# vwxyzjn/cleanrl

Hardware: NVIDIA H100
Metric: env steps/sec (SPS) PPO Breakout num_envs=1024 (higher is better)
Workload: dtype bf16

## Files before the change

cleanrl_b200/csrc/tc_conv1_u8.cuh:

```cuda
#pragma once
#include "tc_base.cuh"
#include <cuda_fp16.h>
#include "tc_conv_win.cuh"

namespace b200rl {
using namespace tc;

__device__ __forceinline__ uint64_t desc_kmajor_sw64(uint32_t smem_addr) {
    return (uint64_t)((smem_addr & 0x3FFFFu) >> 4) | (1ull << 16) | (32ull << 32) | kDescSwizzle64;
}
__device__ __forceinline__ uint64_t desc_mnmajor_sw64(uint32_t smem_addr, uint32_t lbo) {
    return (uint64_t)((smem_addr & 0x3FFFFu) >> 4) | ((uint64_t)((lbo >> 4) & 0x3FFF) << 16) | (32ull << 32) | kDescSwizzle64;
}
__device__ __forceinline__ uint32_t img64_off(int r, int c) { return (uint32_t)(r * 64 + ((c ^ ((r >> 1) & 3)) << 4)); }
constexpr int kS2dThreads = 256;
__global__ void __launch_bounds__(kS2dThreads) tc_frames_to_s2d_u8(const uint8_t* __restrict__ obs, const int64_t* __restrict__ rows,
                                                                   int64_t n, uint8_t* __restrict__ out_rm, uint8_t* __restrict__ out_cm) {
    __shared__ __align__(16) uint8_t frame[28224];
    const int64_t i = blockIdx.x;
    const int64_t img = rows ? rows[i] : i;
    const int4* src = reinterpret_cast<const int4*>(obs + img * 28224);
#pragma unroll
    for (int k = 0; k < 7; ++k) {
        const int t = threadIdx.x + k * kS2dThreads;
        if (t < 1764) reinterpret_cast<int4*>(frame)[t] = __ldg(src + t);
    }
    __syncthreads();
    int4* rm = reinterpret_cast<int4*>(out_rm + i * 441 * 64);
    for (int t = threadIdx.x; t < 441 * 4; t += kS2dThreads) {
        const int pos = t >> 2, c = t & 3;
        const int Y = (pos * 3121) >> 16, X = pos - Y * 21;
        const uint8_t* p = frame + c * 7056 + (Y * 4) * 84 + X * 4;
        int4 v;
        v.x = *reinterpret_cast<const int*>(p); v.y = *reinterpret_cast<const int*>(p + 84);
        v.z = *reinterpret_cast<const int*>(p + 168); v.w = *reinterpret_cast<const int*>(p + 252);
        rm[t] = v;
    }
    uint8_t* cm = out_cm + i * 64 * 448;
    for (int t = threadIdx.x; t < 16 * 112; t += kS2dThreads) {
        const int g = t / 112, q = t - g * 112;
        const uint8_t* prow = frame + (g >> 2) * 7056 + (g & 3) * 84;
        uint32_t w[4];
#pragma unroll
        for (int e = 0; e < 4; ++e) {
            const int pos = q * 4 + e, pc = pos < 441 ? pos : 440;
            const int Y = (pc * 3121) >> 16, X = pc - Y * 21;
            const uint32_t v = *reinterpret_cast<const uint32_t*>(prow + (Y * 4) * 84 + X * 4);
            w[e] = pos < 441 ? v : 0u;
        }
        const uint32_t lo01 = __byte_perm(w[0], w[1], 0x5140), hi01 = __byte_perm(w[0], w[1], 0x7362);
        const uint32_t lo23 = __byte_perm(w[2], w[3], 0x5140), hi23 = __byte_perm(w[2], w[3], 0x7362);
        uint32_t* dst = reinterpret_cast<uint32_t*>(cm + (g * 4) * 448) + q;
        dst[0] = __byte_perm(lo01, lo23, 0x5410);
        dst[112] = __byte_perm(lo01, lo23, 0x7632);
        dst[224] = __byte_perm(hi01, hi23, 0x5410);
        dst[336] = __byte_perm(hi01, hi23, 0x7632);
    }
}

__global__ void __launch_bounds__(256) tc_pack_conv1_i8(const float* __restrict__ w, int8_t* __restrict__ limbs, float* __restrict__ sc) {
    __shared__ float red[32];
    const int co = blockIdx.x, idx = threadIdx.x;
    const float v = w[co * 256 + idx];
    float m = fabsf(v);
#pragma unroll
    for (int o = 16; o > 0; o >>= 1) m = fmaxf(m, __shfl_xor_sync(0xffffffffu, m, o));
    if ((idx & 31) == 0) red[idx >> 5] = m;
    __syncthreads();
    float mx = red[0];
#pragma unroll
    for (int k = 1; k < 8; ++k) mx = fmaxf(mx, red[k]);
    const float s = mx > 0.f ? mx * (128.0f / 127.0f) : 1.0f;
    const float u = v / s * 128.0f;
    float l1 = rintf(u);
    l1 = fminf(fmaxf(l1, -127.f), 127.f);
    float l2 = rintf((u - l1) * 128.0f);
    l2 = fminf(fmaxf(l2, -127.f), 127.f);
    const int kx = idx & 7, ky = (idx >> 3) & 7, c = idx >> 6;
    const int a = ky >> 2, sy = ky & 3, b = kx >> 2, sx = kx & 3;
    const int k = (a * 2 + b) * 64 + c * 16 + sy * 4 + sx;
    limbs[co * 256 + k] = (int8_t)l1;
    limbs[(32 + co) * 256 + k] = (int8_t)l2;
    if (idx == 0) {
        sc[co] = s / 128.0f / 255.0f;
        sc[32 + co] = s / 16384.0f / 255.0f;
    }
}

struct Conv1U8Params {
    const int64_t* rows;
    int n;
    int64_t n_images;
    const int8_t* limbs;
    const float* sc;
    const float* bias;
    bf16* out;
    uint32_t* mask_out;
};

constexpr int kConv1I8Threads = 384;
template <int STAGES>
__global__ void __launch_bounds__(kConv1I8Threads, 1) tc_conv1_i8(const __grid_constant__ CUtensorMap tmA, const __grid_constant__ CUtensorMap tmW,
                                                                   const Conv1U8Params p, int total_tiles) {
    constexpr int BN = 64, WR = 144, NTAPS = 4;
    constexpr int STAGE_BYTES = WR * 128;
    constexpr int B_CHUNK = BN * 64;
    extern __shared__ uint8_t smem_raw[];
    __shared__ uint64_t full_bar[STAGES], empty_bar[STAGES], w_bar;
    __shared__ __align__(16) float s_sc[32], s_bias[32];
    uint8_t* smem = reinterpret_cast<uint8_t*>((reinterpret_cast<uintptr_t>(smem_raw) + 1023) & ~uintptr_t(1023));
    const int tid = threadIdx.x, warp = tid >> 5;
    uint8_t* sW = smem;
    uint8_t* sRing = smem + NTAPS * B_CHUNK;

    if (tid == 0) {
        for (int s = 0; s < STAGES; ++s) { mbar_init(&full_bar[s], 1); mbar_init(&empty_bar[s], 8); }
        mbar_init(&w_bar, 1);
        fence_barrier_init();
        tma_prefetch_desc(&tmA);
        tma_prefetch_desc(&tmW);
    }
    if (tid < 32) { s_sc[tid] = p.sc[32 + tid]; s_bias[tid] = p.bias[tid]; }
    __syncthreads();
    const int tile_begin = (int)(((int64_t)total_tiles * blockIdx.x) / gridDim.x);
    const int tile_end = (int)(((int64_t)total_tiles * (blockIdx.x + 1)) / gridDim.x);

    if (warp == 0) {
        if (tid == 0) {
            uint32_t q = 0;
            int z_next = 0;
            if (tile_begin < tile_end) {
                const int img = tile_begin >> 1;
                z_next = p.rows ? (int)__ldg(p.rows + img) : img;
            }
            for (int tile = tile_begin; tile < tile_end; ++tile, ++q) {
                const uint32_t s = q % STAGES;
                const int z = z_next;
                if (tile + 1 < tile_end) {
                    const int img = (tile + 1) >> 1;
                    z_next = p.rows ? (int)__ldg(p.rows + img) : img;
                }
                if (q >= (uint32_t)STAGES) mbar_wait(&empty_bar[s], ((q / STAGES) - 1) & 1);
                mbar_arrive_expect_tx(&full_bar[s], (uint32_t)STAGE_BYTES);
                tma_load_3d(smem_u32(sRing + (size_t)s * STAGE_BYTES), &tmA, 0, (tile & 1) * 128, z, &full_bar[s]);
                if (q == 0) {
                    mbar_arrive_expect_tx(&w_bar, (uint32_t)(NTAPS * B_CHUNK));
#pragma unroll
                    for (int t = 0; t < NTAPS; ++t) tma_load_3d(smem_u32(sW + t * B_CHUNK), &tmW, t * 64, 0, 0, &w_bar);
                }
            }
        }
    } else if (warp >= 4) {
        const int wg = (warp - 4) >> 2, wt = tid & 127, lane = tid & 31, qd = lane & 3;
        const uint32_t w_base = smem_u32(sW);
        constexpr int off[4] = {0, 1, 21, 22};
        int acc[2][32];
#pragma unroll
        for (int e = 0; e < 2; ++e)
#pragma unroll
            for (int c = 0; c < 32; ++c) acc[e][c] = 0;
        if (tile_begin < tile_end) mbar_wait(&w_bar, 0);
        for (int tile = tile_begin; tile < tile_end; ++tile) {
            const uint32_t q = (uint32_t)(tile - tile_begin), s = q % STAGES;
            mbar_wait(&full_bar[s], (q / STAGES) & 1);
            wgmma_fence();
            const uint32_t win = smem_u32(sRing + (size_t)s * STAGE_BYTES) + (uint32_t)(wg * 64 * 128);
#pragma unroll
            for (int e = 0; e < 2; ++e) {
#pragma unroll
                for (int t = 0; t < NTAPS; ++t) {
                    const int po = e + off[t];
                    const uint64_t a = desc_kmajor(win + (uint32_t)((po >> 1) * 128 + (po & 1) * 64));
                    const uint64_t b = desc_kmajor_sw64(w_base + (uint32_t)(t * B_CHUNK));
#pragma unroll
                    for (int kk = 0; kk < 2; ++kk) wgmma_u8s8_n64(acc[e], a + 2 * kk, b + 2 * kk, (t | kk) != 0 ? 1u : 0u);
                }
            }
            wgmma_commit();
            wgmma_wait<0>();
            wgmma_fence_operands(acc[0]);
            wgmma_fence_operands(acc[1]);
            if (lane == 0) mbar_arrive(&empty_bar[s]);
            const int i = tile >> 1;
#pragma unroll
            for (int e = 0; e < 2; ++e) {
#pragma unroll
                for (int hr = 0; hr < 2; ++hr) {
                    const int lrow = wg * 64 + ((wt >> 5) << 4) + (lane >> 2) + 8 * hr;
                    const int rem = 2 * (((tile & 1) << 7) + lrow) + e;
                    const int Y = (rem * 3121) >> 16, X = rem - Y * 21;
                    const bool valid = rem < 441 && Y < 20 && X < 20;
                    const int64_t cell = ((int64_t)i * 10 + (Y >> 1)) * 10 + (X >> 1);
                    const int cls = (Y & 1) * 2 + (X & 1);
                    uint32_t bits = 0u, pk[4];
#pragma unroll
                    for (int j = 0; j < 4; ++j) {
                        const int co = 8 * j + 2 * qd;
                        const float f0 = fmaf((float)(acc[e][4 * j + 2 * hr] * 128 + acc[e][4 * (j + 4) + 2 * hr]), s_sc[co], s_bias[co]);
                        const float f1 = fmaf((float)(acc[e][4 * j + 2 * hr + 1] * 128 + acc[e][4 * (j + 4) + 2 * hr + 1]), s_sc[co + 1],
                                              s_bias[co + 1]);
                        bits |= (f0 > 0.f ? 1u : 0u) << co;
                        bits |= (f1 > 0.f ? 1u : 0u) << (co + 1);
                        pk[j] = pack_bf16x2_relu(f0, f1);
                    }
                    bits |= __shfl_xor_sync(0xffffffffu, bits, 1);
                    bits |= __shfl_xor_sync(0xffffffffu, bits, 2);
                    if (valid) {
                        if (qd == 0) p.mask_out[cell * 4 + cls] = bits;
                        uint32_t* dst = reinterpret_cast<uint32_t*>(reinterpret_cast<uint8_t*>(p.out) + (cell * 4 + cls) * 64);
#pragma unroll
                        for (int j = 0; j < 4; ++j) dst[4 * j + qd] = pk[j];
                    }
                }
            }
        }
    }
}

struct Conv21BwdU8Params {
    const int64_t* rows;
    int n;
    int64_t rows_per_cta;
    const bf16* w2dg;
    const uint32_t* m1;
    float* ws;
    float* wsb;
};
constexpr int kC1WXStages = 4, kC21WinStages = 2;
constexpr int kC1WXRows = 33, kC1WXBytes = kC1WXRows * 128, kC1WF16Bytes = 136 * 128;
constexpr int kC1WYBytes = 128 * 64, kC1WYPadRows = 24, kC1WYPad = kC1WYPadRows * 64;
constexpr int kC1WShift = 21;
constexpr int kC21WinRows = 140, kC21WinBytes = 18 * 1024;
constexpr int kC21W2Bytes = 4 * 128 * 128;
constexpr int kC21ImgBytes = kC1WYPad + 4 * kC1WYBytes;
constexpr int kC21MaskBytes = 100 * 16;
constexpr size_t kC21Smem = (size_t)kC21W2Bytes + (size_t)kC21WinStages * (kC21WinBytes + kC21MaskBytes) + 2 * (size_t)kC21ImgBytes +
                            2 * (size_t)kC1WF16Bytes + (size_t)kC1WXStages * kC1WXBytes + 1024;
static_assert(kC21Smem + 4608 <= 227 * 1024, "conv21_bwd: shared memory exceeds 227 KB");
static_assert((kC21W2Bytes + kC21WinStages * kC21WinBytes + 2 * kC21ImgBytes) % 1024 == 0, "the fp16 images need 1 KB alignment");
constexpr float kDact1Scale = 4096.0f;

__device__ __forceinline__ uint32_t prmt(uint32_t a, uint32_t b, uint32_t sel) {
    uint32_t d;
    asm("prmt.b32 %0, %1, %2, %3;" : "=r"(d) : "r"(a), "r"(b), "r"(sel));
    return d;
}
constexpr float kU8Bias = 1024.0f;
__device__ __forceinline__ void u8x16_to_f16_biased(const uint4& v, uint4& lo, uint4& hi) {
    constexpr uint32_t k64 = 0x64646464u;
    lo = make_uint4(prmt(v.x, k64, 0x5140u), prmt(v.x, k64, 0x7362u), prmt(v.y, k64, 0x5140u), prmt(v.y, k64, 0x7362u));
    hi = make_uint4(prmt(v.z, k64, 0x5140u), prmt(v.z, k64, 0x7362u), prmt(v.w, k64, 0x5140u), prmt(v.w, k64, 0x7362u));
}
__device__ __forceinline__ uint4 lds128(uint32_t addr) {
    uint4 v;
    asm volatile("ld.shared.v4.u32 {%0, %1, %2, %3}, [%4];" : "=r"(v.x), "=r"(v.y), "=r"(v.z), "=r"(v.w) : "r"(addr) : "memory");
    return v;
}
__device__ __forceinline__ void sts128(uint32_t addr, const uint4& v) {
    asm volatile("st.shared.v4.u32 [%0], {%1, %2, %3, %4};" ::"r"(addr), "r"(v.x), "r"(v.y), "r"(v.z), "r"(v.w) : "memory");
}
__device__ __forceinline__ uint32_t pack_f16x2_sat(float lo, float hi) {
    uint32_t d;
    asm("cvt.rn.satfinite.f16x2.f32 %0, %1, %2;" : "=r"(d) : "f"(hi), "f"(lo));
    return d;
}

__device__ __forceinline__ void sts32(uint32_t addr, uint32_t v) { asm volatile("st.shared.u32 [%0], %1;" ::"r"(addr), "r"(v) : "memory"); }
__device__ __forceinline__ void tma_store_3d(const void* tmap, uint32_t smem_src, int x, int y, int z) {
    asm volatile("cp.async.bulk.tensor.3d.global.shared::cta.bulk_group [%0, {%1, %2, %3}], [%4];"
                 ::"l"(reinterpret_cast<uint64_t>(tmap)), "r"(x), "r"(y), "r"(z), "r"(smem_src) : "memory");
}
__device__ __forceinline__ void bulk_commit() { asm volatile("cp.async.bulk.commit_group;" ::: "memory"); }
template <int N> __device__ __forceinline__ void bulk_wait_read() { asm volatile("cp.async.bulk.wait_group.read %0;" ::"n"(N) : "memory"); }
template <int N> __device__ __forceinline__ void bulk_wait() { asm volatile("cp.async.bulk.wait_group %0;" ::"n"(N) : "memory"); }
__device__ __forceinline__ void bulk_load(uint32_t smem_dst, const void* src, uint32_t bytes, uint64_t* bar) {
    asm volatile("cp.async.bulk.shared::cluster.global.mbarrier::complete_tx::bytes [%0], [%1], %2, [%3];"
                 ::"r"(smem_dst), "l"(src), "r"(bytes), "r"(smem_u32(bar)) : "memory");
}

constexpr int kC1WThreads = 512;
__global__ void __launch_bounds__(kC1WThreads, 1) tc_conv21_bwd_u8(const __grid_constant__ CUtensorMap tmX, const __grid_constant__ CUtensorMap tmWin,
                                                                 const __grid_constant__ CUtensorMap tmY, const Conv21BwdU8Params p) {
    constexpr int XS = kC1WXStages, WS = kC21WinStages;
    extern __shared__ uint8_t smem_raw[];
    __shared__ uint64_t xfull[XS], xempty[XS], wfull[WS], wempty[WS], yfull[2], yempty[2], ffull[2], fempty[2];
    __shared__ float sRed[32 * 32], sBias[32];
    uint8_t* smem = reinterpret_cast<uint8_t*>((reinterpret_cast<uintptr_t>(smem_raw) + 1023) & ~uintptr_t(1023));
    uint8_t* sW2 = smem;
    uint8_t* sWin = sW2 + kC21W2Bytes;
    uint8_t* sImg = sWin + (size_t)WS * kC21WinBytes;
    uint8_t* sF = sImg + 2 * (size_t)kC21ImgBytes;
    uint8_t* sX = sF + 2 * (size_t)kC1WF16Bytes;
    uint8_t* sM = sX + (size_t)XS * kC1WXBytes;
    const int tid = threadIdx.x, warp = tid >> 5, lane = tid & 31;
    if (tid == 0) {
        for (int s = 0; s < XS; ++s) { mbar_init(&xfull[s], 1); mbar_init(&xempty[s], 4); }
        for (int s = 0; s < WS; ++s) { mbar_init(&wfull[s], 1); mbar_init(&wempty[s], 4); }
        for (int s = 0; s < 2; ++s) {
            mbar_init(&yfull[s], 1); mbar_init(&yempty[s], 4);
            mbar_init(&ffull[s], 4); mbar_init(&fempty[s], 4);
        }
        fence_barrier_init();
        tma_prefetch_desc(&tmX);
        tma_prefetch_desc(&tmWin);
        tma_prefetch_desc(&tmY);
    }
    for (int idx = tid; idx < 4 * 128 * 8; idx += blockDim.x) {
        const int c16 = idx & 7, r = (idx >> 3) & 127, t = idx >> 10;
        *reinterpret_cast<int4*>(sW2 + t * (128 * 128) + img_off(r, c16)) = ldg16(p.w2dg + r * 256 + t * 64 + c16 * 8);
    }
    for (int idx = tid; idx < 2 * kC21ImgBytes / 16; idx += blockDim.x) reinterpret_cast<int4*>(sImg)[idx] = make_int4(0, 0, 0, 0);
    fence_proxy_async_smem();
    __syncthreads();
    const int64_t M = (int64_t)p.n * 512;
    const int64_t m_begin = (int64_t)blockIdx.x * p.rows_per_cta;
    int64_t m_end = m_begin + p.rows_per_cta;
    if (m_end > M) m_end = M;
    const int nsteps = (int)((m_end - m_begin) >> 7);
    const int nimg = nsteps >> 2;
    const int img0 = (int)(m_begin >> 9);

    if (warp < 4) {
        if (warp == 0 && lane == 0) {
            auto image_of = [&](int j) -> int { return p.rows ? (int)__ldg(p.rows + img0 + j) : img0 + j; };
            int z = 0, z_next = image_of(0);
            for (int k = 0; k < nsteps; ++k) {
                if ((k & 3) == 0) {
                    z = z_next;
                    if ((k >> 2) + 1 < nimg) z_next = image_of((k >> 2) + 1);
                }
#pragma unroll
                for (int hb = 0; hb < 2; ++hb) {
                    const int j = 2 * k + hb, xs = j % XS;
                    if (j >= XS) mbar_wait(&xempty[xs], ((j / XS) - 1) & 1);
                    mbar_arrive_expect_tx(&xfull[xs], (uint32_t)kC1WXBytes);
                    tma_load_3d(smem_u32(sX + (size_t)xs * kC1WXBytes), &tmX, 0, (k & 3) * 64 + hb * 32, z, &xfull[xs]);
                }
            }
        } else if (warp == 1 && lane == 0) {
            for (int j = 0; j < nimg; ++j) {
                const int s = j % WS;
                if (j >= WS) mbar_wait(&wempty[s], ((j / WS) - 1) & 1);
                mbar_arrive_expect_tx(&wfull[s], (uint32_t)(kC21WinRows * 128 + kC21MaskBytes));
                tma_load_2d(smem_u32(sWin + (size_t)s * kC21WinBytes), &tmWin, 0, (img0 + j) * 121, &wfull[s]);
                bulk_load(smem_u32(sM + (size_t)s * kC21MaskBytes), p.m1 + (int64_t)(img0 + j) * 100 * 4, (uint32_t)kC21MaskBytes, &wfull[s]);
            }
        }
    } else if (warp < 8) {
        const int wt = tid - 128, lane4 = lane >> 2, qd = lane & 3;
        const uint32_t w_base = smem_u32(sW2);
        const int rq = wt >> 2, c16 = wt & 3;
        float bsum[8];
#pragma unroll
        for (int e = 0; e < 8; ++e) bsum[e] = 0.f;
        for (int j = 0; j < nimg; ++j) {
            const int i = img0 + j, buf = j & 1, s = j % WS;
            const uint32_t img = smem_u32(sImg + (size_t)buf * kC21ImgBytes) + kC1WYPad;
            const uint32_t masks = smem_u32(sM + (size_t)s * kC21MaskBytes);
            mbar_wait(&wfull[s], (j / WS) & 1);
            if (j >= 2) mbar_wait(&yempty[buf], ((j >> 1) - 1) & 1);
            if (wt == 0) bulk_wait_read<1>();
            named_bar(1, 128);
#pragma unroll 1
            for (int h2 = 0; h2 < 2; ++h2) {
                float d[64];
                wgmma_fence();
                const uint32_t win = smem_u32(sWin + (size_t)s * kC21WinBytes) + (uint32_t)(h2 * 64 * 128);
                constexpr int shift[4] = {12, 11, 1, 0};
#pragma unroll
                for (int t = 0; t < 4; ++t) {
                    const uint64_t a = desc_kmajor(win + (uint32_t)shift[t] * 128u);
                    const uint64_t b = desc_kmajor(w_base + (uint32_t)(t * 128 * 128));
#pragma unroll
                    for (int kk = 0; kk < 4; ++kk) WgmmaBf16<128, 0, 0>::mma(d, a + 2 * kk, b + 2 * kk, (t | kk) != 0 ? 1u : 0u);
                }
                wgmma_commit();
                int pos[2];
                uint4 mb[2];
#pragma unroll
                for (int hr = 0; hr < 2; ++hr) {
                    const int r = h2 * 64 + ((wt >> 5) << 4) + lane4 + 8 * hr;
                    const int Y = (r * 5958) >> 16, X = r - Y * 11;
                    const bool valid = Y < 10 && X < 10;
                    pos[hr] = valid ? 2 * Y * 21 + 2 * X : -1;
                    mb[hr] = make_uint4(0u, 0u, 0u, 0u);
                    if (valid) mb[hr] = lds128(masks + (uint32_t)(Y * 10 + X) * 16u);
                }
                wgmma_wait<0>();
                wgmma_fence_operands(d);
#pragma unroll
                for (int hr = 0; hr < 2; ++hr) {
                    if (pos[hr] < 0) continue;
                    const uint32_t mw[4] = {mb[hr].x, mb[hr].y, mb[hr].z, mb[hr].w};
#pragma unroll
                    for (int jj = 0; jj < 16; ++jj) {
                        const int g = jj >> 2, c = 8 * (jj & 3) + 2 * qd;
                        float f0 = d[4 * jj + 2 * hr] * kDact1Scale, f1 = d[4 * jj + 2 * hr + 1] * kDact1Scale;
                        if (!((mw[g] >> c) & 1u)) f0 = 0.f;
                        if (!((mw[g] >> (c + 1)) & 1u)) f1 = 0.f;
                        const int q = pos[hr] + (g >> 1) * 21 + (g & 1);
                        sts32(img + img64_off(q, c >> 3) + (uint32_t)((c & 7) * 2), pack_f16x2_sat(f0, f1));
                    }
                }
                __syncwarp();
                if (h2 == 1 && lane == 0) mbar_arrive(&wempty[s]);
            }
            fence_proxy_async_smem();
            named_bar(1, 128);
            if (wt == 0) {
                mbar_arrive(&yfull[buf]);
#pragma unroll
                for (int k = 0; k < 4; ++k) tma_store_3d(&tmY, img + (uint32_t)(k * kC1WYBytes), 0, k * 128, i);
                bulk_commit();
            }
#pragma unroll 1
            for (int st = 0; st < 4; ++st) {
#pragma unroll
                for (int ps = 0; ps < 4; ++ps) {
                    const uint4 v = lds128(img + (uint32_t)(st * kC1WYBytes) + img64_off(ps * 32 + rq, c16));
                    const uint32_t w[4] = {v.x, v.y, v.z, v.w};
#pragma unroll
                    for (int e = 0; e < 4; ++e) {
                        const float2 f = __half22float2(*reinterpret_cast<const __half2*>(&w[e]));
                        bsum[2 * e] += f.x;
                        bsum[2 * e + 1] += f.y;
                    }
                }
            }
        }
        if (wt == 0) bulk_wait<0>();
#pragma unroll
        for (int e = 0; e < 8; ++e) sRed[rq * 32 + c16 * 8 + e] = bsum[e];
        named_bar(1, 128);
        if (wt < 32) {
            float t = 0.f;
#pragma unroll
            for (int l = 0; l < 32; ++l) t += sRed[l * 32 + wt];
            p.wsb[(int64_t)blockIdx.x * 64 + wt] = t;
            sBias[wt] = t * kU8Bias;
        }
        named_bar(2, 256);
    } else if (warp < 12) {
        const int wt = tid & 127, qd = lane & 3;
        float d[64];
#pragma unroll
        for (int e = 0; e < 64; ++e) d[e] = 0.f;
        auto step = [&](int it) {
            const int fs = it & 1, buf = (it >> 2) & 1;
            if ((it & 3) == 0) mbar_wait(&yfull[buf], (it >> 3) & 1);
            mbar_wait(&ffull[fs], (it >> 1) & 1);
            wgmma_fence();
            const uint32_t ystep = smem_u32(sImg + (size_t)buf * kC21ImgBytes) + (uint32_t)(kC1WYPad + (it & 3) * kC1WYBytes);
            const uint64_t ad = desc_mnmajor_sw64(ystep - kC1WShift * 64, kC1WShift * 64);
            const uint64_t bd = desc_mnmajor(smem_u32(sF + (size_t)fs * kC1WF16Bytes), 128);
#pragma unroll
            for (int kk = 0; kk < 8; ++kk) WgmmaF16N128<1, 1>::mma(d, ad + 64 * kk, bd + 128 * kk, (it | kk) != 0 ? 1u : 0u);
            wgmma_commit();
        };
        for (int it = 0; it + 1 < nsteps; ++it) {
            step(it);
            wgmma_wait<1>();
            if (it > 0 && lane == 0) {
                mbar_arrive(&fempty[(it - 1) & 1]);
                if (((it - 1) & 3) == 3) mbar_arrive(&yempty[((it - 1) >> 2) & 1]);
            }
        }
        step(nsteps - 1);
        wgmma_wait<0>();
        wgmma_fence_operands(d);
        named_bar(2, 256);
        const int m = ((wt >> 5) << 4) + (lane >> 2), b = m < 32 ? 1 : 0, co = m & 31;
        const float bias0 = sBias[co], bias8 = sBias[co + 8];
        float* wsc = p.ws + (int64_t)blockIdx.x * 256 * 64;
#pragma unroll
        for (int j = 0; j < 16; ++j) {
            const int h = j >> 3, c = 8 * (j & 7) + 2 * qd;
            float* q = wsc + (int64_t)((2 * b + h) * 64 + c) * 64 + co;
            q[0] = d[4 * j] - bias0;
            q[64] = d[4 * j + 1] - bias0;
            q[8] = d[4 * j + 2] - bias8;
            q[64 + 8] = d[4 * j + 3] - bias8;
        }
    } else {
        const int wt = tid & 127;
        for (int it = 0; it < nsteps; ++it) {
            const int fs = it & 1;
            const uint32_t img = smem_u32(sF + (size_t)fs * kC1WF16Bytes);
            if (it >= 2) mbar_wait(&fempty[fs], ((it >> 1) - 1) & 1);
#pragma unroll
            for (int hb = 0; hb < 2; ++hb) {
                const int j = 2 * it + hb, xs = j % XS;
                const uint32_t blk = smem_u32(sX + (size_t)xs * kC1WXBytes);
                const int nch = (64 + hb) * 4;
                mbar_wait(&xfull[xs], (j / XS) & 1);
                uint4 v[3];
#pragma unroll
                for (int i = 0; i < 2 + hb; ++i)
                    if (wt + 128 * i < nch) v[i] = lds128(blk + (uint32_t)(wt + 128 * i) * 16u);
#pragma unroll
                for (int i = 0; i < 2 + hb; ++i) {
                    const int t = wt + 128 * i;
                    if (t < nch) {
                        const int r = 64 * hb + (t >> 2), c = t & 3;
                        uint4 lo, hi;
                        u8x16_to_f16_biased(v[i], lo, hi);
                        sts128(img + (uint32_t)(r * 128 + (((2 * c) ^ (r & 7)) << 4)), lo);
                        sts128(img + (uint32_t)(r * 128 + (((2 * c + 1) ^ (r & 7)) << 4)), hi);
                    }
                }
                __syncwarp();
                if (lane == 0) mbar_arrive(&xempty[xs]);
            }
            fence_proxy_async_smem();
            __syncwarp();
            if (lane == 0) mbar_arrive(&ffull[fs]);
        }
    }
}

static int launch_conv21_bwd_u8(const Conv21BwdU8Params& p, const void* frames_rm, int64_t n_images, const bf16* dact2b, void* dact1_f16,
                                int ctas, cudaStream_t s, const char* what) {
    int rc;
    if (p.rows_per_cta % 512 != 0) return fail(B200RL_ERR_INVALID_ARGUMENT, "%s: a CTA must own whole images (512 grid rows)", what);
    if (ctas < 1 || (int64_t)(ctas - 1) * p.rows_per_cta >= (int64_t)p.n * 512)
        return fail(B200RL_ERR_INVALID_ARGUMENT, "%s: every CTA must own at least one image", what);
    CUtensorMap tmX, tmWin, tmY;
    memset(&tmX, 0, sizeof(tmX)); memset(&tmWin, 0, sizeof(tmWin)); memset(&tmY, 0, sizeof(tmY));
    if ((rc = make_tmap_pairs_u8(&tmX, frames_rm, n_images, kC1WXRows, false, what))) return rc;
    if ((rc = make_tmap_2d(&tmWin, dact2b, (int64_t)p.n * 121, 64, kC21WinRows, what))) return rc;
    if ((rc = make_tmap_3d_u8(&tmY, dact1_f16, p.n, 441, 64, 64, 128, 64, what))) return rc;
    static SmemAttrCache attr;
    if ((rc = attr.ensure(tc_conv21_bwd_u8, kC21Smem, what))) return rc;
    tc_conv21_bwd_u8<<<ctas, kC1WThreads, kC21Smem, s>>>(tmX, tmWin, tmY, p);
    return check_launch(what);
}

constexpr int kConv1I8Stages = 8;
static int launch_conv1_i8(const Conv1U8Params& p, const void* frames_rm, cudaStream_t s, const char* what) {
    constexpr int STAGES = kConv1I8Stages;
    const size_t smem = (size_t)4 * 64 * 64 + (size_t)STAGES * 144 * 128 + 1024;
    const int total = p.n * 2;
    int grid = num_sms();
    if (grid > total) grid = total;
    CUtensorMap tmA, tmW;
    memset(&tmA, 0, sizeof(tmA));
    memset(&tmW, 0, sizeof(tmW));
    int rc = make_tmap_pairs_u8(&tmA, frames_rm, p.n_images, 144, true, what);
    if (rc) return rc;
    if ((rc = make_tmap_3d_u8(&tmW, p.limbs, 1, 64, 256, 256, 64, 64, what))) return rc;
    static SmemAttrCache attr;
    if ((rc = attr.ensure(tc_conv1_i8<STAGES>, smem, what))) return rc;
    tc_conv1_i8<STAGES><<<grid, kConv1I8Threads, smem, s>>>(tmA, tmW, p, total);
    return check_launch(what);
}

}
```

Measured before the change: 1.441 million.

## Overlap conv1 wgmma with epilogue via ping-pong accumulators and vectorized stores

```diff
diff --git a/cleanrl_b200/csrc/tc_conv1_u8.cuh b/cleanrl_b200/csrc/tc_conv1_u8.cuh
--- a/cleanrl_b200/csrc/tc_conv1_u8.cuh
+++ b/cleanrl_b200/csrc/tc_conv1_u8.cuh
@@ -154,65 +154,105 @@
         const int wg = (warp - 4) >> 2, wt = tid & 127, lane = tid & 31, qd = lane & 3;
         const uint32_t w_base = smem_u32(sW);
         constexpr int off[4] = {0, 1, 21, 22};
-        int acc[2][32];
-#pragma unroll
-        for (int e = 0; e < 2; ++e)
-#pragma unroll
-            for (int c = 0; c < 32; ++c) acc[e][c] = 0;
-        if (tile_begin < tile_end) mbar_wait(&w_bar, 0);
-        for (int tile = tile_begin; tile < tile_end; ++tile) {
-            const uint32_t q = (uint32_t)(tile - tile_begin), s = q % STAGES;
-            mbar_wait(&full_bar[s], (q / STAGES) & 1);
-            wgmma_fence();
+        int acc0[32], acc1[32];
+#pragma unroll
+        for (int c = 0; c < 32; ++c) acc0[c] = acc1[c] = 0;
+        wgmma_fence_operands(acc0);
+        wgmma_fence_operands(acc1);
+        auto issue = [&](int (&acc)[32], int e, uint32_t s) {
             const uint32_t win = smem_u32(sRing + (size_t)s * STAGE_BYTES) + (uint32_t)(wg * 64 * 128);
 #pragma unroll
-            for (int e = 0; e < 2; ++e) {
-#pragma unroll
-                for (int t = 0; t < NTAPS; ++t) {
-                    const int po = e + off[t];
-                    const uint64_t a = desc_kmajor(win + (uint32_t)((po >> 1) * 128 + (po & 1) * 64));
-                    const uint64_t b = desc_kmajor_sw64(w_base + (uint32_t)(t * B_CHUNK));
-#pragma unroll
-                    for (int kk = 0; kk < 2; ++kk) wgmma_u8s8_n64(acc[e], a + 2 * kk, b + 2 * kk, (t | kk) != 0 ? 1u : 0u);
-                }
+            for (int t = 0; t < NTAPS; ++t) {
+                const int po = e + off[t];
+                const uint64_t a = desc_kmajor(win + (uint32_t)((po >> 1) * 128 + (po & 1) * 64));
+                const uint64_t b = desc_kmajor_sw64(w_base + (uint32_t)(t * B_CHUNK));
+#pragma unroll
+                for (int kk = 0; kk < 2; ++kk) wgmma_u8s8_n64(acc, a + 2 * kk, b + 2 * kk, (t | kk) != 0 ? 1u : 0u);
             }
             wgmma_commit();
-            wgmma_wait<0>();
-            wgmma_fence_operands(acc[0]);
-            wgmma_fence_operands(acc[1]);
-            if (lane == 0) mbar_arrive(&empty_bar[s]);
-            const int i = tile >> 1;
-#pragma unroll
-            for (int e = 0; e < 2; ++e) {
+        };
+        float sc[8], bias[8];
+#pragma unroll
+        for (int k = 0; k < 8; ++k) {
+            sc[k] = s_sc[8 * (k >> 1) + 2 * qd + (k & 1)];
+            bias[k] = s_bias[8 * (k >> 1) + 2 * qd + (k & 1)];
+        }
+        int slot[2][2][2];
+#pragma unroll
+        for (int tp = 0; tp < 2; ++tp)
+#pragma unroll
+            for (int e = 0; e < 2; ++e)
 #pragma unroll
                 for (int hr = 0; hr < 2; ++hr) {
                     const int lrow = wg * 64 + ((wt >> 5) << 4) + (lane >> 2) + 8 * hr;
-                    const int rem = 2 * (((tile & 1) << 7) + lrow) + e;
+                    const int rem = 2 * ((tp << 7) + lrow) + e;
                     const int Y = (rem * 3121) >> 16, X = rem - Y * 21;
                     const bool valid = rem < 441 && Y < 20 && X < 20;
-                    const int64_t cell = ((int64_t)i * 10 + (Y >> 1)) * 10 + (X >> 1);
-                    const int cls = (Y & 1) * 2 + (X & 1);
-                    uint32_t bits = 0u, pk[4];
-#pragma unroll
-                    for (int j = 0; j < 4; ++j) {
-                        const int co = 8 * j + 2 * qd;
-                        const float f0 = fmaf((float)(acc[e][4 * j + 2 * hr] * 128 + acc[e][4 * (j + 4) + 2 * hr]), s_sc[co], s_bias[co]);
-                        const float f1 = fmaf((float)(acc[e][4 * j + 2 * hr + 1] * 128 + acc[e][4 * (j + 4) + 2 * hr + 1]), s_sc[co + 1],
-                                              s_bias[co + 1]);
-                        bits |= (f0 > 0.f ? 1u : 0u) << co;
-                        bits |= (f1 > 0.f ? 1u : 0u) << (co + 1);
-                        pk[j] = pack_bf16x2_relu(f0, f1);
-                    }
-                    bits |= __shfl_xor_sync(0xffffffffu, bits, 1);
-                    bits |= __shfl_xor_sync(0xffffffffu, bits, 2);
-                    if (valid) {
-                        if (qd == 0) p.mask_out[cell * 4 + cls] = bits;
-                        uint32_t* dst = reinterpret_cast<uint32_t*>(reinterpret_cast<uint8_t*>(p.out) + (cell * 4 + cls) * 64);
-#pragma unroll
-                        for (int j = 0; j < 4; ++j) dst[4 * j + qd] = pk[j];
-                    }
-                }
-            }
+                    slot[tp][e][hr] = valid ? ((Y >> 1) * 10 + (X >> 1)) * 4 + (Y & 1) * 2 + (X & 1) : -1;
+                }
+        auto epilogue = [&](const int (&acc)[32], int e, int tile) {
+            uint32_t* const mimg = p.mask_out + (int64_t)(tile >> 1) * 400;
+            uint4* const oimg = reinterpret_cast<uint4*>(p.out) + (int64_t)(tile >> 1) * 1600;
+#pragma unroll
+            for (int hr = 0; hr < 2; ++hr) {
+                const int sl = (tile & 1) ? slot[1][e][hr] : slot[0][e][hr];
+                uint32_t bits = 0u, pk[4];
+#pragma unroll
+                for (int j = 0; j < 4; ++j) {
+                    const float f0 = fmaf((float)(acc[4 * j + 2 * hr] * 128 + acc[4 * (j + 4) + 2 * hr]), sc[2 * j], bias[2 * j]);
+                    const float f1 = fmaf((float)(acc[4 * j + 2 * hr + 1] * 128 + acc[4 * (j + 4) + 2 * hr + 1]), sc[2 * j + 1],
+                                          bias[2 * j + 1]);
+                    bits |= (f0 > 0.f ? 1u << (8 * j) : 0u) | (f1 > 0.f ? 2u << (8 * j) : 0u);
+                    pk[j] = pack_bf16x2_relu(f0, f1);
+                }
+                bits <<= 2 * qd;
+                bits |= __shfl_xor_sync(0xffffffffu, bits, 1);
+                bits |= __shfl_xor_sync(0xffffffffu, bits, 2);
+                const bool hi = (qd & 2) != 0, odd = (qd & 1) != 0;
+#pragma unroll
+                for (int k = 0; k < 2; ++k) {
+                    const uint32_t r = __shfl_xor_sync(0xffffffffu, hi ? pk[k] : pk[k + 2], 2);
+                    if (hi) pk[k] = r; else pk[k + 2] = r;
+                }
+#pragma unroll
+                for (int k = 0; k < 4; k += 2) {
+                    const uint32_t r = __shfl_xor_sync(0xffffffffu, odd ? pk[k] : pk[k + 1], 1);
+                    if (odd) pk[k] = r; else pk[k + 1] = r;
+                }
+                if (sl >= 0) {
+                    if (qd == 0) mimg[sl] = bits;
+                    oimg[sl * 4 + qd] = make_uint4(pk[0], pk[1], pk[2], pk[3]);
+                }
+            }
+        };
+        if (tile_begin < tile_end) {
+            mbar_wait(&w_bar, 0);
+            mbar_wait(&full_bar[0], 0);
+            wgmma_fence();
+            issue(acc0, 0, 0);
+            issue(acc1, 1, 0);
+            for (int tile = tile_begin; tile + 1 < tile_end; ++tile) {
+                const uint32_t q = (uint32_t)(tile - tile_begin), s = q % STAGES, sn = (q + 1) % STAGES;
+                wgmma_wait<1>();
+                wgmma_fence_operands(acc0);
+                epilogue(acc0, 0, tile);
+                mbar_wait(&full_bar[sn], ((q + 1) / STAGES) & 1);
+                wgmma_fence();
+                issue(acc0, 0, sn);
+                wgmma_wait<1>();
+                wgmma_fence_operands(acc1);
+                if (lane == 0) mbar_arrive(&empty_bar[s]);
+                epilogue(acc1, 1, tile);
+                wgmma_fence();
+                issue(acc1, 1, sn);
+            }
+            const int tile = tile_end - 1;
+            wgmma_wait<1>();
+            wgmma_fence_operands(acc0);
+            epilogue(acc0, 0, tile);
+            wgmma_wait<0>();
+            wgmma_fence_operands(acc1);
+            epilogue(acc1, 1, tile);
         }
     }
 }
```

Measured after the change: 1.478 million (median of 6 runs). 2.6% higher.
